# C-bowman/inference-tools

Hardware: AMD Instinct MI355X
Metric: GpRegressor fit+predict wall-time and GFLOP/s at N=16384, d=8; % fp64 MFMA peak (higher is better)
Workload: dtype f64

## Files before the change

inference-tools_amd/csrc/api.hip:

```cpp
#include "api_internal.h"
#include <malloc.h>


thread_local std::string g_create_err;


int lane_streams(gpmi_ctx* c, Lane& L) {
  const size_t index = c->lanes.size() - 1;
  L.owns_stream = index < 2;
  if (!L.owns_stream) L.stream = c->lanes[index % 2].stream;
  if (L.owns_stream) HIPCHK(c, hipStreamCreateWithFlags(&L.stream, hipStreamNonBlocking));
  hipDeviceProp_t prop;
  HIPCHK(c, hipGetDeviceProperties(&prop, c->device));
  c->ncu = prop.multiProcessorCount;
  HIPCHK(c, hipEventCreateWithFlags(&L.ev_la, hipEventDisableTiming));
  HIPCHK(c, hipEventCreateWithFlags(&L.ev_panel, hipEventDisableTiming));
  HIPCHK(c, hipEventCreateWithFlags(&L.ev_join, hipEventDisableTiming));
  HIPCHK(c, hipEventCreateWithFlags(&L.ev_main, hipEventDisableTiming));
  HIPCHK(c, hipEventCreateWithFlags(&L.ev_slice, hipEventDisableTiming));
  return L.panel_flags.alloc_zeroed(c, GPMI_PANEL_FL_INTS);
}


bool ensure_masked_pair(gpmi_ctx* c, Lane& L, int k) {
// ... 264 lines not shown
  } else {
    launch_lml_reduce(s, L.vec, L.A, c->ld, c->np, L.red + 2 * slot);
  }
  HIPCHK(c, hipGetLastError());
  return GPMI_OK;
}

int ensure_second_matrix(gpmi_ctx* c, Lane& L) {
  return L.B2 ? GPMI_OK : L.B2.alloc(c, c->np * c->ld);
}

int ensure_inv2(gpmi_ctx* c, Lane& F, hipStream_t s) {
  if (F.inv2_valid) return GPMI_OK;
  const int64_t nob = (c->np / GPMI_NB + 3) / 4;
  if (!F.inv2)
    if (int rc = F.inv2.alloc(c, nob * GPMI_OB * GPMI_OB)) return rc;
  if (!F.inv2_t)
    if (int rc = F.inv2_t.alloc(c, nob * 256 * 256)) return rc;
  build_inv2(s, F.A, c->np, c->ld, F.invD, F.inv2, F.inv2_t);
  HIPCHK(c, hipGetLastError());
  F.inv2_valid = true;
  return GPMI_OK;
}

int ensure_trsm_panel(gpmi_ctx* c, int64_t rows) {
  return c->trsm_panel.reserve(c, rows * (GPMI_OB + 32));
}

int enqueue_inverse_factor(gpmi_ctx* c, Lane& L, Lane& F) {
  if (int rc = ensure_inv2(c, F, L.stream)) return rc;
  if (int rc = ensure_trsm_panel(c, c->np)) return rc;
// ... 557 lines not shown
```

inference-tools_amd/csrc/api_linv.hip:

```cpp
#include "api_internal.h"

namespace {

__global__ void linv_add_diag_kernel(double* __restrict__ J, int64_t ld, const double* __restrict__ sig2,
                                     int64_t mp) {
  const int64_t i = (int64_t)blockIdx.x * blockDim.x + threadIdx.x;
  if (i < mp) J[i * ld + i] += sig2[i];
}


int linv_alloc(gpmi_ctx* c, DevBuf<double>& b, int64_t doubles) {
  return b ? GPMI_OK : b.alloc_zeroed(c, doubles);
}

int linv_factor(gpmi_ctx* c, const KParams& p, const double* mu_host, const double* K_host = nullptr) {
  LinvState& S = c->linv;
  Lane& L = c->lanes[0];
  hipStream_t s = L.stream;
  const int nt = (int)(c->np / GPMI_NB), mt = (int)(S.mp / GPMI_NB);
  const int64_t vmax = S.mp > c->np ? S.mp : c->np;
  double* v = S.vec;
  double* r = S.vec + vmax;
  double* mu_dev = S.vec + 2 * vmax;
  double* amu = S.vec + 3 * vmax;
// ... 101 lines not shown
  ARGCHK(c, K_host, "K is NULL");
  return linv_lml_impl(c, KParams{}, K_host, mu, lml, info);
}

static int linv_lml_grad_impl(gpmi_ctx* c, const KParams& p, int n_theta, const double* K_host, const double* mu,
                              double* lml, double* grad_theta, double* trace_q, double* G_host, double* at_alpha,
                              int* info) {
  ARGCHK(c, mu && lml && (grad_theta || G_host), "mu / lml / output is NULL");
  if (int rc = set_device(c)) return rc;
  LinvState& S = c->linv;
  Lane& L = c->lanes[0];
  hipStream_t s = L.stream;
  const int nt = (int)(c->np / GPMI_NB), mt = (int)(S.mp / GPMI_NB);
  const int64_t vmax = S.mp > c->np ? S.mp : c->np;
  if (int rc = linv_alloc(c, S.J2, S.mp * S.ldm)) return rc;
  if (int rc = linv_alloc(c, S.inv2, (int64_t)((mt + 3) / 4) * GPMI_OB * GPMI_OB)) return rc;
  if (int rc = linv_alloc(c, S.inv2_t, (int64_t)((mt + 3) / 4) * 256 * 256)) return rc;
  if (int rc = linv_alloc(c, S.panel, S.mp * (GPMI_OB + 32))) return rc;
  const int64_t need = n_theta >= 0 ? grad_ws_doubles(c->np, n_theta) : 0;
  if (int rc = S.gws.reserve(c, need)) return rc;
  if (int rc = linv_factor(c, p, mu, K_host)) return rc;
  double* v = S.vec;
  double* alpha = S.vec + 4 * vmax;
  double* w = S.vec + 5 * vmax;
  double* gout = L.red + 16;
  trsv_backward(c, s, S.J, S.mp, S.ldm, S.invD, v, alpha, L.info);
  launch_rows_dot(s, S.At, S.ldm, c->np, S.mp, alpha, w);
  build_inv2(s, S.J, S.mp, S.ldm, S.invD, S.inv2, S.inv2_t);
  launch_set_identity(s, S.J2, S.ldm, S.mp);
  trsm_rows_forward(c, s, S.J, S.mp, S.ldm, S.inv2, S.J2, S.mp, true, nullptr, S.panel);
  launch_gemm(s, TILES_LOWER, OP_ASSIGN, false, 1, S.J, S.ldm, S.J2, S.ldm, S.J2, S.ldm, mt, mt, (int)S.mp);
// ... 38 lines not shown
  ARGCHK(c, K_host && G_host, "K / G is NULL");
  return linv_lml_grad_impl(c, KParams{}, -1, K_host, mu, lml, nullptr, nullptr, G_host, at_alpha, info);
}

static int linv_posterior_impl(gpmi_ctx* c, const KParams& p, const double* K_host, const double* mu, double* mean,
                               double* cov, int* info) {
  ARGCHK(c, mu && mean, "mu / mean is NULL");
  if (int rc = set_device(c)) return rc;
  LinvState& S = c->linv;
  Lane& L = c->lanes[0];
  hipStream_t s = L.stream;
  const int nt = (int)(c->np / GPMI_NB), mt = (int)(S.mp / GPMI_NB);
  const int64_t vmax = S.mp > c->np ? S.mp : c->np;
  if (int rc = linv_alloc(c, S.Q, c->np * S.ldm)) return rc;
  if (int rc = linv_alloc(c, S.X, c->np * S.ldm)) return rc;
  if (int rc = linv_alloc(c, S.inv2, (int64_t)((mt + 3) / 4) * GPMI_OB * GPMI_OB)) return rc;
  if (int rc = linv_alloc(c, S.inv2_t, (int64_t)((mt + 3) / 4) * 256 * 256)) return rc;
  if (int rc = linv_factor(c, p, mu, K_host)) return rc;
  double* v = S.vec;
  double* dm = S.vec + 5 * vmax;
  build_inv2(s, S.J, S.mp, S.ldm, S.invD, S.inv2, S.inv2_t);
  launch_gemm_nt(s, TILES_RECT, OP_ASSIGN, S.Q, S.ldm, S.K, c->ld, S.A, c->ld, nt, mt, (int)c->np);
  trsm_rows_forward(c, s, S.J, S.mp, S.ldm, S.inv2, S.Q, c->np, false, S.X, nullptr);
  launch_rows_dot(s, S.X, S.ldm, c->np, S.mp, v, dm);
  if (cov) launch_gemm_nt(s, TILES_RECT, OP_SUB, S.K, c->ld, S.X, S.ldm, S.X, S.ldm, nt, nt, (int)S.mp);
  HIPCHK(c, hipGetLastError());
  HIPCHK(c, hipMemcpyAsync(L.h_info, L.info, sizeof(int), hipMemcpyDeviceToHost, s));
  HIPCHK(c, hipMemcpyAsync(mean, dm, sizeof(double) * c->n, hipMemcpyDeviceToHost, s));
  if (cov)
    HIPCHK(c, hipMemcpy2DAsync(cov, sizeof(double) * c->n, S.K, sizeof(double) * c->ld, sizeof(double) * c->n,
                               c->n, hipMemcpyDeviceToHost, s));
// ... 28 lines not shown
```

inference-tools_amd/csrc/gemm_f64.hip:

```cpp
#include <cstdlib>

#include "gemm_tiles.h"

namespace {

using namespace gemm_tiles;

struct GemmArgs {
  double* C;
  const double* A;
  const double* B;
  int64_t ldc, lda, ldb;
  int ntr, ntc, k;
  int kskip;
  unsigned long long* stamp;
  int64_t sC, sA, sB;
  int split, tile_base;
  int zlocal_tiles;
  int mixed_full;
};

struct WgId {
  int wid;
  int64_t bz;
};
__device__ inline int xcd_remap(int b, int nwg);
__device__ inline WgId wg_id(int kskip, int zlocal_tiles) {
  if (zlocal_tiles > 0) {
    const int n = (int)blockIdx.x, m = n >> 3;
    return {m % zlocal_tiles, (int64_t)(m / zlocal_tiles) * 8 + (n & 7)};
  }
  return {kskip ? (int)blockIdx.x : xcd_remap(blockIdx.x, gridDim.x), (int64_t)blockIdx.z};
}

// ... 53 lines not shown
    tile_of<TILES>(g.tile_base + wid, g.ntr, g.ntc, ti, tj);
    if (TILES == TILES_RECT && (g.kskip == 2 || g.kskip == 4) && 2 * ti >= g.ntr) tj = g.ntc - 1 - tj;
  }

  const int tid = threadIdx.x;
  const bool stamp_first = g.stamp && tid == 0 && blockIdx.x < 8 && blockIdx.z == 0;
  if (stamp_first) g.stamp[blockIdx.x] = __builtin_amdgcn_s_memrealtime();
  const unsigned mid = gridDim.x >> 1;
  const bool stamp_clock = g.stamp && tid == 0 && blockIdx.x >= mid && blockIdx.x < mid + 8 && blockIdx.z == 0;
  unsigned long long c_start = 0, r_start = 0;
  if (stamp_clock) {
    r_start = __builtin_amdgcn_s_memrealtime();
    c_start = __builtin_amdgcn_s_memtime();
  }
  const int kbeg = (g.kskip == 1) ? ti * BM : (g.kskip == 4) ? tj * BN : 0;
  const int kend = (g.kskip == 2 && (tj + 1) * BN < g.k) ? (tj + 1) * BN : g.k;
  const int64_t bz = me.bz;
  const double* __restrict__ Ag = g.A + bz * g.sA + (int64_t)ti * BM * g.lda + kbeg;
  const double* __restrict__ Bg = BKN ? g.B + bz * g.sB + (int64_t)kbeg * g.ldb + (int64_t)tj * BN
                                      : g.B + bz * g.sB + (int64_t)tj * BN * g.ldb + kbeg;
  double* Cg = g.C + bz * g.sC + (int64_t)ti * BM * g.ldc + (int64_t)tj * BN;
  if constexpr (OP == OP_ASSIGN && BKN == 0 && BN == 128 && BM <= 64) {
    if (g.kskip == 3) {
      staged_tile<OP, BKN, BM, BN, CST_NT, true>(Ag, Bg, Cg, g.lda, g.ldb, g.ldc, (kend - kbeg) / BK, smem);
    } else {
      staged_tile<OP, BKN, BM, BN>(Ag, Bg, Cg, g.lda, g.ldb, g.ldc, (kend - kbeg) / BK, smem);
    }
  } else {
    staged_tile<OP, BKN, BM, BN>(Ag, Bg, Cg, g.lda, g.ldb, g.ldc, (kend - kbeg) / BK, smem);
  }

// ... 10 lines not shown

#ifndef GPMI_DMA_WGS
#define GPMI_DMA_WGS 2
#endif
typedef __attribute__((address_space(3))) double gemm_lds_double_t;
typedef __attribute__((address_space(1))) double gemm_glb_double_t;
template <int OP>
__device__ __attribute__((noinline)) void dma64_quarter(const gemm_glb_double_t* Ag, const gemm_glb_double_t* Bg,
                                                        gemm_glb_double_t* Cg, int64_t lda, int64_t ldb, int64_t ldc, int nk,
                                                        gemm_lds_double_t* smem) {
  gemm_lds_double_t* su = (gemm_lds_double_t*)(uintptr_t)(unsigned)__builtin_amdgcn_readfirstlane((int)(unsigned)(uintptr_t)smem);
  dma64_tile<OP>((const double*)Ag, (const double*)Bg, (double*)Cg, lda, ldb, ldc, __builtin_amdgcn_readfirstlane(nk),
                 (double*)su);
}

template <int TILES, int OP>
__global__ __launch_bounds__(256, GPMI_DMA_WGS) void gemm_dma_kernel(GemmArgs g) {
  __shared__ double smem[DMA128_LDS_DOUBLES];
  int ti, tj;
  if (g.mixed_full > 0 && (int)blockIdx.x >= g.mixed_full) {
    const int w = xcd_remap((int)blockIdx.x - g.mixed_full, (int)gridDim.x - g.mixed_full);
    tile_of<TILES>(g.tile_base + g.mixed_full + (w >> 2), g.ntr, g.ntc, ti, tj);
    const int r0 = 64 * ((w >> 1) & 1), c0 = 64 * (w & 1);
    const double* Aq = g.A + ((int64_t)ti * 128 + r0) * g.lda;
    const double* Bq = g.B + ((int64_t)tj * 128 + c0) * g.ldb;
    double* Cq = g.C + ((int64_t)ti * 128 + r0) * g.ldc + (int64_t)tj * 128 + c0;
    dma64_quarter<OP>((const gemm_glb_double_t*)Aq, (const gemm_glb_double_t*)Bq, (gemm_glb_double_t*)Cq, g.lda, g.ldb, g.ldc,
                      g.k / DMA_BK, (gemm_lds_double_t*)smem);
    if (g.stamp && threadIdx.x == 0) {
      asm volatile("s_waitcnt vmcnt(0)" ::: "memory");
      g.stamp[8 + (__builtin_amdgcn_s_getreg(((4 - 1) << 11) | 20) & 7)] = __builtin_amdgcn_s_memrealtime();
    }
    return;
  }
  WgId me = wg_id(g.kskip, g.zlocal_tiles);
  if (g.mixed_full > 0) me.wid = xcd_remap((int)blockIdx.x, g.mixed_full);
  tile_of<TILES>(g.tile_base + me.wid, g.ntr, g.ntc, ti, tj);
  const int tid = threadIdx.x;
  const bool stamp_first = g.stamp && tid == 0 && blockIdx.x < 8 && blockIdx.z == 0;
  if (stamp_first) g.stamp[blockIdx.x] = __builtin_amdgcn_s_memrealtime();
  const unsigned mid = gridDim.x >> 1;
  const bool stamp_clock = g.stamp && tid == 0 && blockIdx.x >= mid && blockIdx.x < mid + 8;
  unsigned long long c_start = 0, r_start = 0;
  if (stamp_clock) {
    r_start = __builtin_amdgcn_s_memrealtime();
    c_start = __builtin_amdgcn_s_memtime();
  }
  const int kbeg = (g.kskip == 1) ? ti * 128 : 0;
  const int kend = (g.kskip == 2 && (tj + 1) * 128 < g.k) ? (tj + 1) * 128 : g.k;
  const int64_t bz = me.bz;
  const double* __restrict__ Ag = g.A + bz * g.sA + (int64_t)ti * 128 * g.lda + kbeg;
// ... 2 lines not shown
  dma128_tile<OP>(Ag, Bg, Cg, g.lda, g.ldb, g.ldc, (kend - kbeg) / DMA_BK, smem);
  const bool stamp_end = g.stamp && tid == 0 && blockIdx.x + 1024 >= gridDim.x;
  if (stamp_end) {
    asm volatile("s_waitcnt vmcnt(0)" ::: "memory");
    g.stamp[8 + (__builtin_amdgcn_s_getreg(((4 - 1) << 11) | 20) & 7)] = __builtin_amdgcn_s_memrealtime();
  }
  if (stamp_clock)
    g.stamp[16 + blockIdx.x - mid] = ((__builtin_amdgcn_s_memtime() - c_start) << 32) |
                                     ((__builtin_amdgcn_s_memrealtime() - r_start) & 0xffffffffull);
}

template <int TILES, int OP>
__global__ __launch_bounds__(256, 4) void gemm_dma64_kernel(GemmArgs g) {
  __shared__ double smem[DMA64_LDS_DOUBLES];
  int ti, tj;
  const WgId me = wg_id(g.kskip, g.zlocal_tiles);
  const int wid = me.wid;
  if (g.split) {
    int bi, bj;
    tile_of<TILES>(g.tile_base + (wid >> 2), g.ntr >> 1, g.ntc >> 1, bi, bj);
    ti = 2 * bi + ((wid >> 1) & 1);
    tj = 2 * bj + (wid & 1);
  } else {
    tile_of<TILES>(g.tile_base + wid, g.ntr, g.ntc, ti, tj);
  }
  const int tid = threadIdx.x;
  const bool stamp_first = g.stamp && tid == 0 && blockIdx.x < 8;
  if (stamp_first) g.stamp[blockIdx.x] = __builtin_amdgcn_s_memrealtime();
  const int kbeg = (g.kskip == 1) ? ti * 64 : 0;
  const int kend = (g.kskip == 2 && (tj + 1) * 64 < g.k) ? (tj + 1) * 64 : g.k;
  const int64_t bz = me.bz;
  const double* __restrict__ Ag = g.A + bz * g.sA + (int64_t)ti * 64 * g.lda + kbeg;
  const double* __restrict__ Bg = g.B + bz * g.sB + (int64_t)tj * 64 * g.ldb + kbeg;
  double* Cg = g.C + bz * g.sC + (int64_t)ti * 64 * g.ldc + (int64_t)tj * 64;
  dma64_tile<OP>(Ag, Bg, Cg, g.lda, g.ldb, g.ldc, (kend - kbeg) / DMA_BK, smem);
  const bool stamp_end = g.stamp && tid == 0 && blockIdx.x + 2048 >= gridDim.x;
  if (stamp_end) {
    asm volatile("s_waitcnt vmcnt(0)" ::: "memory");
    g.stamp[8 + (__builtin_amdgcn_s_getreg(((4 - 1) << 11) | 20) & 7)] = __builtin_amdgcn_s_memrealtime();
  }
}

}

namespace {
void launch_gemm_part(hipStream_t s, GemmTiles tiles, GemmOp op, bool b_kmajor, int kskip, double* C,
                      int64_t ldc, const double* A, int64_t lda, const double* B, int64_t ldb, int ntr,
                      int ntc, int k, unsigned long long* stamp, const GemmBatch& bt, int part, int64_t nfull,
                      int64_t nend = -1) {
  if (ntr <= 0 || ntc <= 0 || k <= 0) return;
  if (tiles == TILES_LOWER && ntc > ntr) ntc = ntr;
  const int64_t big = (tiles == TILES_RECT) ? (int64_t)ntr * ntc
                                            : (int64_t)ntc * (ntc + 1) / 2 + (int64_t)(ntr - ntc) * ntc;
  int bm = 128, bn = 128;
  static const int64_t BIG_MIN = [] {
    const char* e = std::getenv("GPMI_BIG_MIN");
    return (int64_t)(e ? std::atoi(e) : 384);
  }();
  static const int64_t SMALL_M32_MAX = [] {
    const char* e = std::getenv("GPMI_M32_MAX");
    return (int64_t)(e ? std::atoi(e) : 192);
  }();
  const int64_t m32_max = bt.ncu_hint > 0 ? SMALL_M32_MAX * bt.ncu_hint / 256 : SMALL_M32_MAX;
  const bool small = part == 0 && ((k <= 128) || (big * bt.count < BIG_MIN));
// ... 28 lines not shown
             bt.sC, bt.sA, bt.sB, part == 2 ? 1 : 0, (part == 2 || part == 3) ? (int)nfull : 0, 0, 0};
  int64_t nwg;
  if (tiles == TILES_RECT)
    nwg = (int64_t)g.ntr * g.ntc;
  else
    nwg = (int64_t)g.ntc * (g.ntc + 1) / 2 + (int64_t)(g.ntr - g.ntc) * g.ntc;
  if (part == 1) nwg = nfull;
  if (nend < 0 || nend > big) nend = big;
  if (part == 2) nwg = 4 * (nend - nfull);
  if (part == 3) nwg = nend - nfull;
  if (part == 4) {
    g.mixed_full = (int)nfull;
    nwg = nfull + 4 * (nend - nfull);
  }
  if (nwg <= 0) return;
  dim3 grid((unsigned)nwg, 1, (unsigned)bt.count), block(256);
  static const bool batch_xcd = [] {
    const char* e = std::getenv("GPMI_BATCH_XCD");
    return !e || std::atoi(e) != 0;
  }();
  if (batch_xcd && bt.count >= 8 && bt.count % 8 == 0 && !stamp && nwg * bt.count < (int64_t)1 << 30) {
    g.zlocal_tiles = (int)nwg;
    grid = dim3((unsigned)(nwg * bt.count), 1, 1);
  }
  static const bool no_dma = std::getenv("GPMI_GEMM_NO_DMA") != nullptr;
  if (!no_dma && bm == 128 && bn == 128 && !b_kmajor && part != 2 && k % 128 == 0) {
    if (tiles == TILES_RECT) {
      if (op == OP_SUB) hipLaunchKernelGGL((gemm_dma_kernel<TILES_RECT, OP_SUB>), grid, block, 0, s, g);
      else hipLaunchKernelGGL((gemm_dma_kernel<TILES_RECT, OP_ASSIGN>), grid, block, 0, s, g);
    } else {
      if (op == OP_SUB) hipLaunchKernelGGL((gemm_dma_kernel<TILES_LOWER, OP_SUB>), grid, block, 0, s, g);
      else hipLaunchKernelGGL((gemm_dma_kernel<TILES_LOWER, OP_ASSIGN>), grid, block, 0, s, g);
    }
    return;
  }
  static const bool no_dma64 = std::getenv("GPMI_GEMM_NO_DMA64") != nullptr;
  static const int dma64_min_k = [] {
    const char* e = std::getenv("GPMI_DMA64_MIN_K");
    return e ? std::atoi(e) : 128;
  }();
  if (!no_dma && !no_dma64 && bm == 64 && bn == 64 && !b_kmajor && k % 64 == 0 && k >= dma64_min_k) {
    if (tiles == TILES_RECT) {
      if (op == OP_SUB) hipLaunchKernelGGL((gemm_dma64_kernel<TILES_RECT, OP_SUB>), grid, block, 0, s, g);
      else hipLaunchKernelGGL((gemm_dma64_kernel<TILES_RECT, OP_ASSIGN>), grid, block, 0, s, g);
    } else {
      if (op == OP_SUB) hipLaunchKernelGGL((gemm_dma64_kernel<TILES_LOWER, OP_SUB>), grid, block, 0, s, g);
      else hipLaunchKernelGGL((gemm_dma64_kernel<TILES_LOWER, OP_ASSIGN>), grid, block, 0, s, g);
    }
    return;
  }
#define GPMI_LAUNCH(T, O, B, M, N) \
  hipLaunchKernelGGL((gemm_nt_kernel<T, O, B, M, N>), grid, block, 0, s, g)
  if (bm == 128) {
    if (tiles == TILES_RECT) {
      if (op == OP_SUB) {
        if (b_kmajor) GPMI_LAUNCH(TILES_RECT, OP_SUB, 1, 128, 128); else GPMI_LAUNCH(TILES_RECT, OP_SUB, 0, 128, 128);
// ... 43 lines not shown
  }();
  if (k <= 128 || T < BIG_MIN || ncu <= 0) return T;
  const int64_t rem = T % ncu;
  if (rem == 0 || rem * 100 > (int64_t)ncu * SPLIT_PCT) return T;
  return T - rem;
}

bool gemm_mixed_launches() {
  static const bool mixed = [] {
    const char* e = std::getenv("GPMI_GEMM_MIXED");
    return !e || std::atoi(e) != 0;
  }();
  return mixed;
}

void launch_gemm_nt_split(hipStream_t s, GemmTiles tiles, GemmOp op, double* C, int64_t ldc, const double* A,
                          int64_t lda, const double* B, int64_t ldb, int ntr, int ntc, int k, int64_t nfull,
                          unsigned long long* stamp, unsigned long long* stamp_rest, int64_t nend) {
  if (tiles == TILES_LOWER && ntc > ntr) ntc = ntr;
  const int64_t T = (tiles == TILES_RECT) ? (int64_t)ntr * ntc
                                          : (int64_t)ntc * (ntc + 1) / 2 + (int64_t)(ntr - ntc) * ntc;
  const GemmBatch one{};
  if (nend < 0 || nend > T) nend = T;
  if (nfull >= T) {
    launch_gemm_part(s, tiles, op, false, 0, C, ldc, A, lda, B, ldb, ntr, ntc, k, stamp, one, 0, 0);
    return;
  }
  if (gemm_mixed_launches() && nfull > 0 && nend > nfull && k % 128 == 0 && k > 128) {
    launch_gemm_part(s, tiles, op, false, 0, C, ldc, A, lda, B, ldb, ntr, ntc, k, stamp, one, 4, nfull, nend);
    return;
  }
  launch_gemm_part(s, tiles, op, false, 0, C, ldc, A, lda, B, ldb, ntr, ntc, k, stamp, one, 1, nfull);
  if (nend > nfull)
    launch_gemm_part(s, tiles, op, false, 0, C, ldc, A, lda, B, ldb, ntr, ntc, k, stamp_rest, one, 2, nfull, nend);
}

void launch_gemm_nt_range(hipStream_t s, GemmTiles tiles, GemmOp op, double* C, int64_t ldc, const double* A,
                          int64_t lda, const double* B, int64_t ldb, int ntr, int ntc, int k, int64_t first,
                          int64_t count, unsigned long long* stamp) {
  if (count <= 0) return;
  const GemmBatch one{};
  launch_gemm_part(s, tiles, op, false, 0, C, ldc, A, lda, B, ldb, ntr, ntc, k, stamp, one, 3, first, first + count);
}

void launch_gemm_nt(hipStream_t s, GemmTiles tiles, GemmOp op, double* C, int64_t ldc,
                    const double* A, int64_t lda, const double* B, int64_t ldb, int ntr, int ntc,
                    int k, unsigned long long* stamp, const GemmBatch& bt) {
  launch_gemm(s, tiles, op, false, false, C, ldc, A, lda, B, ldb, ntr, ntc, k, stamp, bt);
}
// ... 1 lines not shown
```

inference-tools_amd/csrc/gemm_tiles.h:

```cpp
#pragma once
#include "gpmi_internal.h"

#ifndef GPMI_C_PLAIN
#define GPMI_C_LOAD(p) __builtin_nontemporal_load(p)
#define GPMI_C_STORE(v, p) __builtin_nontemporal_store(v, p)
#else
#define GPMI_C_LOAD(p) (*(p))
#define GPMI_C_STORE(v, p) (*(p) = (v))
#endif

namespace gemm_tiles {

constexpr int CST_NT = 0, CST_SC1 = 1;
template <int CST>
__device__ __forceinline__ void c_store_begin() {
  if (CST == CST_SC1) asm volatile("s_nop 15\n\ts_nop 15" ::: "memory");
}
template <int CST>
__device__ __forceinline__ void c_store(d2_t v, d2_t* p) {
  if (CST == CST_SC1)
    asm volatile("global_store_dwordx4 %0, %1, off sc1\n\ts_nop 1" ::"v"(p), "v"(v) : "memory");
  else
    GPMI_C_STORE(v, p);
}
// ... 257 lines not shown
    stage(kt + 2);
    stage(kt + 3);
  }
  for (; kt < nk; ++kt) stage(kt);
  c_store_begin<CST>();
#pragma unroll
  for (int i = 0; i < 4; ++i)
#pragma unroll
    for (int jp = 0; jp < 2; ++jp)
#pragma unroll
      for (int r = 0; r < 4; ++r)
        c_store<CST>((d2_t{acc[i][2 * jp][r], acc[i][2 * jp + 1][r]}),
                     reinterpret_cast<d2_t*>(&Cg[(int64_t)(i * 16 + fk + 4 * r) * ldc + jp * 32 + 2 * fr]));
}

template <int OP, int CST = CST_NT>
__device__ __forceinline__ void dma64_tile(const double* __restrict__ Ag, const double* __restrict__ Bg, double* Cg,
                                           int64_t lda, int64_t ldb, int64_t ldc, int nk, double* smem) {
  constexpr int OPD = 64 * DMA_BK;
  const int tid = threadIdx.x, lane = tid & 63, wave = tid >> 6;
  const int wr = wave >> 1, wc = wave & 1;
  const int fr = lane & 15, fk = lane >> 4;
  const int row0 = tid >> 2, slot = tid & 3;
  const int q0 = (slot - 2 * ((row0 >> 2) & 3)) & 3;
  const double* a_src = Ag + (int64_t)row0 * lda + 2 * q0;
  const int bcol = (row0 & 32) + 2 * (row0 & 15) + ((row0 >> 4) & 1);
  const double* b_src = Bg + (int64_t)bcol * ldb + 2 * q0;
  const unsigned lds0 = (unsigned)(uintptr_t)smem;
  const unsigned wave_off = (unsigned)__builtin_amdgcn_readfirstlane(wave * 64 * 16);
  auto issue = [&](int st, int k0) {
    const unsigned base = lds0 + (unsigned)st * (2 * OPD * 8) + wave_off;
    const double* p0 = a_src + k0;
    const double* p1 = b_src + k0;
    asm volatile(
        "s_mov_b32 m0, %2\n\ts_nop 0\n\tglobal_load_lds_dwordx4 %0, off\n\t"
        "s_mov_b32 m0, %3\n\ts_nop 0\n\tglobal_load_lds_dwordx4 %1, off"
        :
        : "v"(p0), "v"(p1), "s"(base), "s"(base + OPD * 8)
        : "memory");
  };
  for (int st = 0; st < DMA_STAGES - 1 && st < nk; ++st) issue(st, st * DMA_BK);

  Cg += (int64_t)(wr * 32) * ldc + wc * 32;
  d4_t acc[2][2];
#pragma unroll
  for (int i = 0; i < 2; ++i)
#pragma unroll
    for (int r = 0; r < 4; ++r) {
// ... 61 lines not shown
```

inference-tools_amd/csrc/gpmi_internal.h:

```cpp
#pragma once
#include <hip/hip_runtime.h>
#include <atomic>
#include <cstdint>
#include <string>
#include <type_traits>
#include <utility>
#include <vector>

#include "gpmi.h"

constexpr int GPMI_NB = 128;
constexpr int GPMI_MAX_D = 64;
constexpr int GPMI_INFO_FLOW_TIMEOUT = -6;
constexpr int GPMI_NPAIRS = 1;

typedef double d2_t __attribute__((ext_vector_type(2)));
typedef double d4_t __attribute__((ext_vector_type(4)));

static inline int64_t round_up(int64_t v, int64_t m) { return (v + m - 1) / m * m; }

struct KParams {
  int kernel;
  int d;
  double a2;
// ... 366 lines not shown
enum GemmOp { OP_SUB = 0, OP_ASSIGN = 1 };
void launch_gemm_nt(hipStream_t s, GemmTiles tiles, GemmOp op, double* C, int64_t ldc,
                    const double* A, int64_t lda, const double* B, int64_t ldb, int ntr, int ntc,
                    int k, unsigned long long* stamp = nullptr, const GemmBatch& bt = GemmBatch());

int64_t gemm_split_point(int64_t T, int ncu, int k);
bool gemm_mixed_launches();
void launch_gemm_nt_split(hipStream_t s, GemmTiles tiles, GemmOp op, double* C, int64_t ldc, const double* A,
                          int64_t lda, const double* B, int64_t ldb, int ntr, int ntc, int k, int64_t nfull,
                          unsigned long long* stamp = nullptr, unsigned long long* stamp_rest = nullptr,
                          int64_t nend = -1);
void launch_gemm_nt_range(hipStream_t s, GemmTiles tiles, GemmOp op, double* C, int64_t ldc, const double* A,
                          int64_t lda, const double* B, int64_t ldb, int ntr, int ntc, int k, int64_t first,
                          int64_t count, unsigned long long* stamp = nullptr);

void launch_gemm(hipStream_t s, GemmTiles tiles, GemmOp op, bool b_kmajor, int kskip, double* C,
                 int64_t ldc, const double* A, int64_t lda, const double* B, int64_t ldb, int ntr,
                 int ntc, int k, unsigned long long* stamp = nullptr, const GemmBatch& bt = GemmBatch());

hipStream_t potrf_first_update_stream(gpmi_ctx* c, Lane& lane, int64_t np, bool allow_lookahead);
void potrf_pair_quiesce(Lane& lane);
void launch_potrf_diag(hipStream_t s, double* Ablk, int64_t ld, double* invD, int* info, int col0,
                       unsigned long long* dbg = nullptr, const BatchShape& bs = BatchShape());
void launch_potrf_diag_fault(hipStream_t s, double* Ablk, int64_t ld, const BatchShape& bs = BatchShape());
void potrf_lower_batched(gpmi_ctx* c, hipStream_t s, double* A, int64_t np, int64_t ld, double* invD,
                         int* info, const BatchShape& bs);
void launch_kbuild_square_batched(hipStream_t s, int kernel, const KParams* pdev, int batch, const double* x,
                                  int64_t n, int64_t np, const double* noise, double* A, int64_t ld,
                                  int64_t stride, int d, int64_t noise_stride = 0);
void potrf_lower(gpmi_ctx* c, Lane& lane, double* A, int64_t np, int64_t ld, double* invD,
// ... 5 lines not shown

bool potrf_flow_enabled(gpmi_ctx* c, Lane& lane, int m);
bool potrf_flow_tail(gpmi_ctx* c, Lane& lane, double* A, int64_t ld, double* invD, int* info, int nt, int t0);
void potrf_flow_free(Lane& lane);

void trsv_forward(gpmi_ctx* c, hipStream_t s, const double* L, int64_t np, int64_t ld,
                  const double* invD, const double* r, double* out, int* err = nullptr,
                  const BatchShape& bs = BatchShape(), bool prefilled = false);
void trsv_backward(gpmi_ctx* c, hipStream_t s, const double* L, int64_t np, int64_t ld,
                   const double* invD, const double* r, double* out, int* err = nullptr,
                   const BatchShape& bs = BatchShape(), bool prefilled = false);
void lane_run_early(Lane& lane, hipStream_t s);
void trsm_identity_batched(hipStream_t s, const double* L, int64_t np, int64_t ld, const double* invD, double* Q,
                           const BatchShape& bs);
constexpr int GPMI_OB = 512;
void build_inv2(hipStream_t s, const double* L, int64_t np, int64_t ld, const double* invD, double* inv2,
                double* tmp);
void trsm_rows_forward(gpmi_ctx* c, hipStream_t s, const double* L, int64_t np, int64_t ld,
                       const double* inv2, double* Q, int64_t mp, bool upper_rhs, double* Qout,
                       double* panel);
void launch_set_identity(hipStream_t s, double* Q, int64_t ld, int64_t np, int batch = 1, int64_t sMat = 0);
void launch_copy(hipStream_t s, const double* src, double* dst, int64_t n);
void launch_copy_rows(hipStream_t s, const double* src, int64_t spitch, double* dst, int64_t dpitch, int64_t width,
                      int64_t height);
void launch_residual(hipStream_t s, const double* y, const double* mu, double mu_const, double* r,
                     int64_t n, int64_t np);
void launch_residual_batched(hipStream_t s, const double* y, const double* mus, const double* mu_consts,
                             double* r, int64_t n, int64_t np, const BatchShape& bs);
void launch_lml_reduce(hipStream_t s, const double* v, const double* L, int64_t ld, int64_t np,
                       double* red, const BatchShape& bs = BatchShape());
// ... 17 lines not shown
```

inference-tools_amd/csrc/solve.hip:

```cpp
#include <cstdlib>
#include <mutex>

#include "gpmi_internal.h"

namespace {

constexpr int NB = GPMI_NB;

__device__ inline double wave_sum(double v) {
#pragma unroll
  for (int off = 32; off > 0; off >>= 1) v += __shfl_down(v, off, 64);
  return v;
}

constexpr unsigned long long FLOW_SENTINEL = 0xFFF8DEADBEEF0000ull;
constexpr int FLOW_THREADS = 512;
constexpr int FLOW_SPIN_LIMIT = 1 << 22;

__device__ inline double flow_poll(const double* p, int* err, bool& dead) {
  const unsigned long long* q = reinterpret_cast<const unsigned long long*>(p);
  unsigned long long bits = __hip_atomic_load(q, __ATOMIC_RELAXED, __HIP_MEMORY_SCOPE_AGENT);
  int spins = 0;
  while (bits == FLOW_SENTINEL && !dead) {
    __builtin_amdgcn_s_sleep(1);
// ... 461 lines not shown
  offdiag(1, 0, 1, 1, (nt - 1 + 3) / 4);
  offdiag(3, 2, 1, 1, (nt - 3 + 3) / 4);
  const int full = nt / 4;
  offdiag(2, 0, 2, 2, full);
  if (nt % 4 == 3) {
    const int64_t b = full;
    const GemmBatch one{};
    const double* Lb = L + (b * 4 * NB) * ld + b * 4 * NB;
    double* Xb = inv2 + b * slot;
    double* Tb = tmp + b * tslot;
    launch_gemm(s, TILES_RECT, OP_ASSIGN, true, 0, Tb, 256, Lb + (int64_t)2 * NB * ld, ld, Xb, GPMI_OB, 1, 2, 2 * NB,
                nullptr, one);
    launch_gemm(s, TILES_RECT, OP_SUB, true, 0, Xb + (int64_t)2 * NB * GPMI_OB, GPMI_OB,
                Xb + (int64_t)2 * NB * GPMI_OB + 2 * NB, GPMI_OB, Tb, 256, 1, 2, NB, nullptr, one);
  }
}

void trsm_rows_forward(gpmi_ctx* c, hipStream_t s, const double* L, int64_t np, int64_t ld,
                       const double* inv2, double* Q, int64_t mp, bool upper_rhs, double* Qout,
                       double* panel) {
  const int nt = (int)(np / NB), mt_all = (int)(mp / NB);
  const int OBT = GPMI_OB / NB;
  const int64_t ldp = GPMI_OB + 32;
  ProfScope ps(c, s, GPMI_PROF_TRSM, (double)mp * np * np, 4.0 * np * np);
  for (int J = 0; J < nt; J += OBT) {
    const int Je = (J + OBT < nt) ? J + OBT : nt;
    const int w = Je - J;
    const int mt = upper_rhs ? (Je < mt_all ? Je : mt_all) : mt_all;
    double* QJ = Q + (int64_t)J * NB;
    double* X = Qout ? Qout + (int64_t)J * NB : panel;
    const int64_t ldx = Qout ? ld : ldp;
    launch_gemm(s, TILES_RECT, OP_ASSIGN, false, 2, X, ldx, QJ, ld, inv2 + (int64_t)(J / OBT) * GPMI_OB * GPMI_OB,
                GPMI_OB, mt, w, w * NB);
    const int rest = nt - Je;
    if (rest > 0)
      launch_gemm_nt_split(s, TILES_RECT, OP_SUB, Q + (int64_t)Je * NB, ld, X, ldx,
                           L + (int64_t)Je * NB * ld + (int64_t)J * NB, ld, mt, rest, w * NB,
                           gemm_split_point((int64_t)mt * rest, c->ncu, w * NB));
    if (!Qout) {
// ... 115 lines not shown
```

Baseline: 55460.

## Couple blocked TRSM steps by fusing next diagonal-block solve into trailing update GEMM

Restructures the blocked forward TRSM so each step's next diagonal-block multiply rides as extra 64x64 link tiles inside the trailing-update GEMM launch. The link tiles use a precomputed coupling matrix G, built in build_inv2 and stored in a doubled inv2 buffer, so the next panel can be produced without waiting for the trailing update to finish. The goal is to shorten the serial critical path and cut the number of kernel launches per block step. In exchange it adds extra precompute GEMMs, doubles the inv2 memory, and introduces new grid-remapping code paths in the DMA GEMM kernels.

```diff
diff --git a/inference-tools_amd/csrc/api.hip b/inference-tools_amd/csrc/api.hip
--- a/inference-tools_amd/csrc/api.hip
+++ b/inference-tools_amd/csrc/api.hip
@@ -302,7 +302,7 @@
   if (F.inv2_valid) return GPMI_OK;
   const int64_t nob = (c->np / GPMI_NB + 3) / 4;
   if (!F.inv2)
-    if (int rc = F.inv2.alloc(c, nob * GPMI_OB * GPMI_OB)) return rc;
+    if (int rc = F.inv2.alloc(c, inv2_doubles(c->np))) return rc;
   if (!F.inv2_t)
     if (int rc = F.inv2_t.alloc(c, nob * 256 * 256)) return rc;
   build_inv2(s, F.A, c->np, c->ld, F.invD, F.inv2, F.inv2_t);
diff --git a/inference-tools_amd/csrc/api_linv.hip b/inference-tools_amd/csrc/api_linv.hip
--- a/inference-tools_amd/csrc/api_linv.hip
+++ b/inference-tools_amd/csrc/api_linv.hip
@@ -139,7 +139,7 @@
   const int nt = (int)(c->np / GPMI_NB), mt = (int)(S.mp / GPMI_NB);
   const int64_t vmax = S.mp > c->np ? S.mp : c->np;
   if (int rc = linv_alloc(c, S.J2, S.mp * S.ldm)) return rc;
-  if (int rc = linv_alloc(c, S.inv2, (int64_t)((mt + 3) / 4) * GPMI_OB * GPMI_OB)) return rc;
+  if (int rc = linv_alloc(c, S.inv2, inv2_doubles(S.mp))) return rc;
   if (int rc = linv_alloc(c, S.inv2_t, (int64_t)((mt + 3) / 4) * 256 * 256)) return rc;
   if (int rc = linv_alloc(c, S.panel, S.mp * (GPMI_OB + 32))) return rc;
   const int64_t need = n_theta >= 0 ? grad_ws_doubles(c->np, n_theta) : 0;
@@ -208,7 +208,7 @@
   const int64_t vmax = S.mp > c->np ? S.mp : c->np;
   if (int rc = linv_alloc(c, S.Q, c->np * S.ldm)) return rc;
   if (int rc = linv_alloc(c, S.X, c->np * S.ldm)) return rc;
-  if (int rc = linv_alloc(c, S.inv2, (int64_t)((mt + 3) / 4) * GPMI_OB * GPMI_OB)) return rc;
+  if (int rc = linv_alloc(c, S.inv2, inv2_doubles(S.mp))) return rc;
   if (int rc = linv_alloc(c, S.inv2_t, (int64_t)((mt + 3) / 4) * 256 * 256)) return rc;
   if (int rc = linv_factor(c, p, mu, K_host)) return rc;
   double* v = S.vec;
diff --git a/inference-tools_amd/csrc/gemm_f64.hip b/inference-tools_amd/csrc/gemm_f64.hip
--- a/inference-tools_amd/csrc/gemm_f64.hip
+++ b/inference-tools_amd/csrc/gemm_f64.hip
@@ -18,6 +18,8 @@
   int split, tile_base;
   int zlocal_tiles;
   int mixed_full;
+  int link_n;
+  GemmLink link;
 };
 
 struct WgId {
@@ -101,7 +103,9 @@
     c_start = __builtin_amdgcn_s_memtime();
   }
   const int kbeg = (g.kskip == 1) ? ti * BM : (g.kskip == 4) ? tj * BN : 0;
-  const int kend = (g.kskip == 2 && (tj + 1) * BN < g.k) ? (tj + 1) * BN : g.k;
+  const int kend = (g.kskip == 2 && (tj + 1) * BN < g.k)   ? (tj + 1) * BN
+                   : (g.kskip == 5 && (ti + 1) * BM < g.k) ? (ti + 1) * BM
+                                                           : g.k;
   const int64_t bz = me.bz;
   const double* __restrict__ Ag = g.A + bz * g.sA + (int64_t)ti * BM * g.lda + kbeg;
   const double* __restrict__ Bg = BKN ? g.B + bz * g.sB + (int64_t)kbeg * g.ldb + (int64_t)tj * BN
@@ -142,12 +146,38 @@
                  (double*)su);
 }
 
+__device__ __attribute__((noinline)) void dma64_link(const gemm_glb_double_t* A1, const gemm_glb_double_t* B1,
+                                                     const gemm_glb_double_t* A2, const gemm_glb_double_t* B2,
+                                                     gemm_glb_double_t* Cg, int64_t lda1, int64_t lda2, int64_t ldc, int nk1,
+                                                     int nk2, gemm_lds_double_t* smem) {
+  gemm_lds_double_t* su = (gemm_lds_double_t*)(uintptr_t)(unsigned)__builtin_amdgcn_readfirstlane((int)(unsigned)(uintptr_t)smem);
+  dma64_tile<OP_ASSIGN, CST_NT, true>((const double*)A1, (const double*)B1, (double*)Cg, lda1, GPMI_OB, ldc,
+                                      __builtin_amdgcn_readfirstlane(nk1), (double*)su, (const double*)A2, (const double*)B2,
+                                      lda2, __builtin_amdgcn_readfirstlane(nk2));
+}
+__device__ __forceinline__ void link_tile(const GemmLink& k, int l, double* smem) {
+  const int tj = k.ntc - 1 - l / k.ntr, ti = l % k.ntr;
+  const double* A1 = k.A1 + (int64_t)ti * 64 * k.lda1;
+  const double* B1 = k.B1 + (int64_t)tj * 64 * GPMI_OB;
+  const double* A2 = k.A2 + (int64_t)ti * 64 * k.lda2;
+  const double* B2 = k.B2 + (int64_t)tj * 64 * GPMI_OB;
+  double* Cl = k.C + (int64_t)ti * 64 * k.ldc + (int64_t)tj * 64;
+  dma64_link((const gemm_glb_double_t*)A1, (const gemm_glb_double_t*)B1, (const gemm_glb_double_t*)A2,
+             (const gemm_glb_double_t*)B2, (gemm_glb_double_t*)Cl, k.lda1, k.lda2, k.ldc, (tj + 1) * 64 / DMA_BK,
+             ti < k.rows2 ? GPMI_OB / DMA_BK : 0, (gemm_lds_double_t*)smem);
+}
+
 template <int TILES, int OP>
 __global__ __launch_bounds__(256, GPMI_DMA_WGS) void gemm_dma_kernel(GemmArgs g) {
   __shared__ double smem[DMA128_LDS_DOUBLES];
   int ti, tj;
+  const int nbulk = (int)gridDim.x - g.link_n;
+  if ((int)blockIdx.x >= nbulk) {
+    link_tile(g.link, (int)blockIdx.x - nbulk, smem);
+    return;
+  }
   if (g.mixed_full > 0 && (int)blockIdx.x >= g.mixed_full) {
-    const int w = xcd_remap((int)blockIdx.x - g.mixed_full, (int)gridDim.x - g.mixed_full);
+    const int w = xcd_remap((int)blockIdx.x - g.mixed_full, nbulk - g.mixed_full);
     tile_of<TILES>(g.tile_base + g.mixed_full + (w >> 2), g.ntr, g.ntc, ti, tj);
     const int r0 = 64 * ((w >> 1) & 1), c0 = 64 * (w & 1);
     const double* Aq = g.A + ((int64_t)ti * 128 + r0) * g.lda;
@@ -163,6 +193,7 @@
   }
   WgId me = wg_id(g.kskip, g.zlocal_tiles);
   if (g.mixed_full > 0) me.wid = xcd_remap((int)blockIdx.x, g.mixed_full);
+  else if (g.link_n > 0) me.wid = xcd_remap((int)blockIdx.x, nbulk);
   tile_of<TILES>(g.tile_base + me.wid, g.ntr, g.ntc, ti, tj);
   const int tid = threadIdx.x;
   const bool stamp_first = g.stamp && tid == 0 && blockIdx.x < 8 && blockIdx.z == 0;
@@ -195,7 +226,13 @@
 __global__ __launch_bounds__(256, 4) void gemm_dma64_kernel(GemmArgs g) {
   __shared__ double smem[DMA64_LDS_DOUBLES];
   int ti, tj;
-  const WgId me = wg_id(g.kskip, g.zlocal_tiles);
+  const int nbulk = (int)gridDim.x - g.link_n;
+  if ((int)blockIdx.x >= nbulk) {
+    link_tile(g.link, (int)blockIdx.x - nbulk, smem);
+    return;
+  }
+  WgId me = wg_id(g.kskip, g.zlocal_tiles);
+  if (g.link_n > 0) me.wid = xcd_remap((int)blockIdx.x, nbulk);
   const int wid = me.wid;
   if (g.split) {
     int bi, bj;
@@ -224,11 +261,24 @@
 
 }
 
+bool gemm_link_supported() {
+  static const bool ok = !std::getenv("GPMI_GEMM_NO_DMA") && !std::getenv("GPMI_GEMM_NO_DMA64");
+  return ok;
+}
+
 namespace {
+void launch_gemm_link(hipStream_t s, const GemmLink& link) {
+  GemmArgs g{};
+  g.link_n = link.ntr * link.ntc;
+  g.link = link;
+  if (g.link_n <= 0) return;
+  hipLaunchKernelGGL((gemm_dma64_kernel<TILES_RECT, OP_ASSIGN>), dim3((unsigned)g.link_n), dim3(256), 0, s, g);
+}
+
 void launch_gemm_part(hipStream_t s, GemmTiles tiles, GemmOp op, bool b_kmajor, int kskip, double* C,
                       int64_t ldc, const double* A, int64_t lda, const double* B, int64_t ldb, int ntr,
                       int ntc, int k, unsigned long long* stamp, const GemmBatch& bt, int part, int64_t nfull,
-                      int64_t nend = -1) {
+                      int64_t nend = -1, const GemmLink* link = nullptr) {
   if (ntr <= 0 || ntc <= 0 || k <= 0) return;
   if (tiles == TILES_LOWER && ntc > ntr) ntc = ntr;
   const int64_t big = (tiles == TILES_RECT) ? (int64_t)ntr * ntc
@@ -287,6 +337,27 @@
     nwg = nfull + 4 * (nend - nfull);
   }
   if (nwg <= 0) return;
+  static const bool no_dma = std::getenv("GPMI_GEMM_NO_DMA") != nullptr;
+  static const bool no_dma64 = std::getenv("GPMI_GEMM_NO_DMA64") != nullptr;
+  static const int dma64_min_k = [] {
+    const char* e = std::getenv("GPMI_DMA64_MIN_K");
+    return e ? std::atoi(e) : 128;
+  }();
+  const bool ring128 = !no_dma && bm == 128 && bn == 128 && !b_kmajor && part != 2 && k % 128 == 0;
+  const bool ring64 = !no_dma && !no_dma64 && bm == 64 && bn == 64 && !b_kmajor && k % 64 == 0 && k >= dma64_min_k;
+  const bool link_rides = link && (ring128 || ring64) && bt.count == 1 && kskip == 0;
+  if (link_rides) {
+    g.link_n = link->ntr * link->ntc;
+    g.link = *link;
+    nwg += g.link_n;
+  }
+  struct LinkBehind {
+    hipStream_t s;
+    const GemmLink* link;
+    ~LinkBehind() {
+      if (link) launch_gemm_link(s, *link);
+    }
+  } link_behind{s, link_rides ? nullptr : link};
   dim3 grid((unsigned)nwg, 1, (unsigned)bt.count), block(256);
   static const bool batch_xcd = [] {
     const char* e = std::getenv("GPMI_BATCH_XCD");
@@ -296,8 +367,7 @@
     g.zlocal_tiles = (int)nwg;
     grid = dim3((unsigned)(nwg * bt.count), 1, 1);
   }
-  static const bool no_dma = std::getenv("GPMI_GEMM_NO_DMA") != nullptr;
-  if (!no_dma && bm == 128 && bn == 128 && !b_kmajor && part != 2 && k % 128 == 0) {
+  if (ring128) {
     if (tiles == TILES_RECT) {
       if (op == OP_SUB) hipLaunchKernelGGL((gemm_dma_kernel<TILES_RECT, OP_SUB>), grid, block, 0, s, g);
       else hipLaunchKernelGGL((gemm_dma_kernel<TILES_RECT, OP_ASSIGN>), grid, block, 0, s, g);
@@ -307,12 +377,7 @@
     }
     return;
   }
-  static const bool no_dma64 = std::getenv("GPMI_GEMM_NO_DMA64") != nullptr;
-  static const int dma64_min_k = [] {
-    const char* e = std::getenv("GPMI_DMA64_MIN_K");
-    return e ? std::atoi(e) : 128;
-  }();
-  if (!no_dma && !no_dma64 && bm == 64 && bn == 64 && !b_kmajor && k % 64 == 0 && k >= dma64_min_k) {
+  if (ring64) {
     if (tiles == TILES_RECT) {
       if (op == OP_SUB) hipLaunchKernelGGL((gemm_dma64_kernel<TILES_RECT, OP_SUB>), grid, block, 0, s, g);
       else hipLaunchKernelGGL((gemm_dma64_kernel<TILES_RECT, OP_ASSIGN>), grid, block, 0, s, g);
@@ -386,25 +451,41 @@
   return mixed;
 }
 
-void launch_gemm_nt_split(hipStream_t s, GemmTiles tiles, GemmOp op, double* C, int64_t ldc, const double* A,
+static void gemm_nt_split(hipStream_t s, GemmTiles tiles, GemmOp op, double* C, int64_t ldc, const double* A,
                           int64_t lda, const double* B, int64_t ldb, int ntr, int ntc, int k, int64_t nfull,
-                          unsigned long long* stamp, unsigned long long* stamp_rest, int64_t nend) {
+                          unsigned long long* stamp, unsigned long long* stamp_rest, int64_t nend, const GemmLink* link) {
   if (tiles == TILES_LOWER && ntc > ntr) ntc = ntr;
   const int64_t T = (tiles == TILES_RECT) ? (int64_t)ntr * ntc
                                           : (int64_t)ntc * (ntc + 1) / 2 + (int64_t)(ntr - ntc) * ntc;
   const GemmBatch one{};
   if (nend < 0 || nend > T) nend = T;
   if (nfull >= T) {
-    launch_gemm_part(s, tiles, op, false, 0, C, ldc, A, lda, B, ldb, ntr, ntc, k, stamp, one, 0, 0);
+    launch_gemm_part(s, tiles, op, false, 0, C, ldc, A, lda, B, ldb, ntr, ntc, k, stamp, one, 0, 0, -1, link);
     return;
   }
   if (gemm_mixed_launches() && nfull > 0 && nend > nfull && k % 128 == 0 && k > 128) {
-    launch_gemm_part(s, tiles, op, false, 0, C, ldc, A, lda, B, ldb, ntr, ntc, k, stamp, one, 4, nfull, nend);
-    return;
-  }
-  launch_gemm_part(s, tiles, op, false, 0, C, ldc, A, lda, B, ldb, ntr, ntc, k, stamp, one, 1, nfull);
+    launch_gemm_part(s, tiles, op, false, 0, C, ldc, A, lda, B, ldb, ntr, ntc, k, stamp, one, 4, nfull, nend, link);
+    return;
+  }
+  launch_gemm_part(s, tiles, op, false, 0, C, ldc, A, lda, B, ldb, ntr, ntc, k, stamp, one, 1, nfull, -1,
+                   nend > nfull ? nullptr : link);
   if (nend > nfull)
-    launch_gemm_part(s, tiles, op, false, 0, C, ldc, A, lda, B, ldb, ntr, ntc, k, stamp_rest, one, 2, nfull, nend);
+    launch_gemm_part(s, tiles, op, false, 0, C, ldc, A, lda, B, ldb, ntr, ntc, k, stamp_rest, one, 2, nfull, nend, link);
+}
+
+void launch_gemm_nt_split(hipStream_t s, GemmTiles tiles, GemmOp op, double* C, int64_t ldc, const double* A,
+                          int64_t lda, const double* B, int64_t ldb, int ntr, int ntc, int k, int64_t nfull,
+                          unsigned long long* stamp, unsigned long long* stamp_rest, int64_t nend) {
+  gemm_nt_split(s, tiles, op, C, ldc, A, lda, B, ldb, ntr, ntc, k, nfull, stamp, stamp_rest, nend, nullptr);
+}
+
+void launch_gemm_nt_split_link(hipStream_t s, double* C, int64_t ldc, const double* A, int64_t lda, const double* B,
+                               int64_t ldb, int ntr, int ntc, int k, int64_t nfull, const GemmLink& link) {
+  if (ntr <= 0 || ntc <= 0) {
+    launch_gemm_link(s, link);
+    return;
+  }
+  gemm_nt_split(s, TILES_RECT, OP_SUB, C, ldc, A, lda, B, ldb, ntr, ntc, k, nfull, nullptr, nullptr, -1, &link);
 }
 
 void launch_gemm_nt_range(hipStream_t s, GemmTiles tiles, GemmOp op, double* C, int64_t ldc, const double* A,
diff --git a/inference-tools_amd/csrc/gemm_tiles.h b/inference-tools_amd/csrc/gemm_tiles.h
--- a/inference-tools_amd/csrc/gemm_tiles.h
+++ b/inference-tools_amd/csrc/gemm_tiles.h
@@ -295,9 +295,11 @@
                      reinterpret_cast<d2_t*>(&Cg[(int64_t)(i * 16 + fk + 4 * r) * ldc + jp * 32 + 2 * fr]));
 }
 
-template <int OP, int CST = CST_NT>
+template <int OP, int CST = CST_NT, bool LINK = false>
 __device__ __forceinline__ void dma64_tile(const double* __restrict__ Ag, const double* __restrict__ Bg, double* Cg,
-                                           int64_t lda, int64_t ldb, int64_t ldc, int nk, double* smem) {
+                                           int64_t lda, int64_t ldb, int64_t ldc, int nk, double* smem,
+                                           const double* __restrict__ Ag2 = nullptr,
+                                           const double* __restrict__ Bg2 = nullptr, int64_t lda2 = 0, int nk2 = 0) {
   constexpr int OPD = 64 * DMA_BK;
   const int tid = threadIdx.x, lane = tid & 63, wave = tid >> 6;
   const int wr = wave >> 1, wc = wave & 1;
@@ -307,12 +309,21 @@
   const double* a_src = Ag + (int64_t)row0 * lda + 2 * q0;
   const int bcol = (row0 & 32) + 2 * (row0 & 15) + ((row0 >> 4) & 1);
   const double* b_src = Bg + (int64_t)bcol * ldb + 2 * q0;
+  const int nk1 = nk;
+  const double* a_src2 = nullptr;
+  const double* b_src2 = nullptr;
+  if (LINK) {
+    a_src2 = Ag2 + (int64_t)row0 * lda2 + 2 * q0 - (int64_t)nk1 * DMA_BK;
+    b_src2 = Bg2 + (int64_t)bcol * ldb + 2 * q0 - (int64_t)nk1 * DMA_BK;
+    nk += nk2;
+  }
   const unsigned lds0 = (unsigned)(uintptr_t)smem;
   const unsigned wave_off = (unsigned)__builtin_amdgcn_readfirstlane(wave * 64 * 16);
   auto issue = [&](int st, int k0) {
     const unsigned base = lds0 + (unsigned)st * (2 * OPD * 8) + wave_off;
-    const double* p0 = a_src + k0;
-    const double* p1 = b_src + k0;
+    const bool second = LINK && k0 >= nk1 * DMA_BK;
+    const double* p0 = (second ? a_src2 : a_src) + k0;
+    const double* p1 = (second ? b_src2 : b_src) + k0;
     asm volatile(
         "s_mov_b32 m0, %2\n\ts_nop 0\n\tglobal_load_lds_dwordx4 %0, off\n\t"
         "s_mov_b32 m0, %3\n\ts_nop 0\n\tglobal_load_lds_dwordx4 %1, off"
diff --git a/inference-tools_amd/csrc/gpmi_internal.h b/inference-tools_amd/csrc/gpmi_internal.h
--- a/inference-tools_amd/csrc/gpmi_internal.h
+++ b/inference-tools_amd/csrc/gpmi_internal.h
@@ -404,6 +404,16 @@
                           int64_t lda, const double* B, int64_t ldb, int ntr, int ntc, int k, int64_t first,
                           int64_t count, unsigned long long* stamp = nullptr);
 
+struct GemmLink {
+  double* C;
+  const double *A1, *B1, *A2, *B2;
+  int64_t ldc, lda1, lda2;
+  int ntr, ntc, rows2;
+};
+bool gemm_link_supported();
+void launch_gemm_nt_split_link(hipStream_t s, double* C, int64_t ldc, const double* A, int64_t lda, const double* B,
+                               int64_t ldb, int ntr, int ntc, int k, int64_t nfull, const GemmLink& link);
+
 void launch_gemm(hipStream_t s, GemmTiles tiles, GemmOp op, bool b_kmajor, int kskip, double* C,
                  int64_t ldc, const double* A, int64_t lda, const double* B, int64_t ldb, int ntr,
                  int ntc, int k, unsigned long long* stamp = nullptr, const GemmBatch& bt = GemmBatch());
@@ -439,6 +449,8 @@
 void trsm_identity_batched(hipStream_t s, const double* L, int64_t np, int64_t ld, const double* invD, double* Q,
                            const BatchShape& bs);
 constexpr int GPMI_OB = 512;
+inline int64_t inv2_doubles(int64_t np) { return 2 * ((np / 128 + 3) / 4) * (int64_t)GPMI_OB * GPMI_OB; }
+bool trsm_coupled();
 void build_inv2(hipStream_t s, const double* L, int64_t np, int64_t ld, const double* invD, double* inv2,
                 double* tmp);
 void trsm_rows_forward(gpmi_ctx* c, hipStream_t s, const double* L, int64_t np, int64_t ld,
diff --git a/inference-tools_amd/csrc/solve.hip b/inference-tools_amd/csrc/solve.hip
--- a/inference-tools_amd/csrc/solve.hip
+++ b/inference-tools_amd/csrc/solve.hip
@@ -499,6 +499,27 @@
     launch_gemm(s, TILES_RECT, OP_SUB, true, 0, Xb + (int64_t)2 * NB * GPMI_OB, GPMI_OB,
                 Xb + (int64_t)2 * NB * GPMI_OB + 2 * NB, GPMI_OB, Tb, 256, 1, 2, NB, nullptr, one);
   }
+  if (nob >= 2 && trsm_coupled()) {
+    double* G = inv2 + (int64_t)nob * slot;
+    (void)hipMemsetAsync(G + slot, 0, (size_t)(nob - 1) * slot * sizeof(double), s);
+    const GemmBatch bg{full - 1, slot, slot, (int64_t)GPMI_OB * ld + GPMI_OB};
+    if (full >= 2)
+      launch_gemm(s, TILES_RECT, OP_SUB, true, 5, G + slot, GPMI_OB, inv2 + slot, GPMI_OB, L + (int64_t)GPMI_OB * ld, ld, 4,
+                  4, GPMI_OB, nullptr, bg);
+    if (nt % 4) {
+      const int64_t b = full;
+      launch_gemm(s, TILES_RECT, OP_SUB, true, 5, G + b * slot, GPMI_OB, inv2 + b * slot, GPMI_OB,
+                  L + (b * GPMI_OB) * ld + (b - 1) * GPMI_OB, ld, nt % 4, 4, (nt % 4) * NB);
+    }
+  }
+}
+
+bool trsm_coupled() {
+  static const bool on = [] {
+    const char* e = std::getenv("GPMI_TRSM_COUPLED");
+    return (!e || std::atoi(e) != 0) && gemm_link_supported();
+  }();
+  return on;
 }
 
 void trsm_rows_forward(gpmi_ctx* c, hipStream_t s, const double* L, int64_t np, int64_t ld,
@@ -508,6 +529,43 @@
   const int OBT = GPMI_OB / NB;
   const int64_t ldp = GPMI_OB + 32;
   ProfScope ps(c, s, GPMI_PROF_TRSM, (double)mp * np * np, 4.0 * np * np);
+  const int nob = (nt + OBT - 1) / OBT;
+  if (nob >= 2 && trsm_coupled()) {
+    const int64_t slot = (int64_t)GPMI_OB * GPMI_OB;
+    const int w0 = OBT < nt ? OBT : nt;
+    int mt_prev = upper_rhs ? (w0 < mt_all ? w0 : mt_all) : mt_all;
+    auto to_q = [&](int J, int w, int mt) {
+      hipLaunchKernelGGL(copy_panel_kernel, dim3((unsigned)(w * NB / 2 / 64), (unsigned)((int64_t)mt * NB)), dim3(64), 0, s,
+                         panel, ldp, Q + (int64_t)J * NB, ld);
+    };
+    launch_gemm(s, TILES_RECT, OP_ASSIGN, false, 2, Qout ? Qout : panel, Qout ? ld : ldp, Q, ld, inv2, GPMI_OB, mt_prev, w0,
+                w0 * NB);
+    if (!Qout) to_q(0, w0, mt_prev);
+    for (int b = 0; b + 1 < nob; ++b) {
+      const int J = b * OBT, Jn = J + OBT;
+      const int Jne = (Jn + OBT < nt) ? Jn + OBT : nt, wn = Jne - Jn;
+      const int mt = upper_rhs ? (Jne < mt_all ? Jne : mt_all) : mt_all;
+      const double* Xb = (Qout ? Qout : Q) + (int64_t)J * NB;
+      GemmLink link;
+      link.C = Qout ? Qout + (int64_t)Jn * NB : panel;
+      link.ldc = Qout ? ld : ldp;
+      link.A1 = Q + (int64_t)Jn * NB;
+      link.lda1 = ld;
+      link.B1 = inv2 + (int64_t)(b + 1) * slot;
+      link.A2 = Xb;
+      link.lda2 = ld;
+      link.B2 = inv2 + (int64_t)(nob + b + 1) * slot;
+      link.ntr = 2 * mt;
+      link.ntc = 2 * wn;
+      link.rows2 = 2 * mt_prev;
+      const int rest = nt - Jne;
+      launch_gemm_nt_split_link(s, Q + (int64_t)Jne * NB, ld, Xb, ld, L + (int64_t)Jne * NB * ld + (int64_t)J * NB, ld,
+                                mt_prev, rest, GPMI_OB, gemm_split_point((int64_t)mt_prev * rest, c->ncu, GPMI_OB), link);
+      if (!Qout) to_q(Jn, wn, mt);
+      mt_prev = mt;
+    }
+    return;
+  }
   for (int J = 0; J < nt; J += OBT) {
     const int Je = (J + OBT < nt) ? J + OBT : nt;
     const int w = Je - J;
```

After: 55160. No clear change (-0.5%).
